# Lightning-AI/lit-llama

Hardware: NVIDIA H100
Metric: LLaMA-7B gptq.int4 decode tokens/sec (higher is better)
Workload: dtype bf16

## Files before the change

### lit-llama_b200/csrc/api.cu

```cuda
#include <algorithm>
#include <cstdlib>
#include <mutex>
#include <utility>
#include <vector>

#include "b2l_common.cuh"

namespace b2l {

extern void* g_attn_timeline;
int decode_step_persistent(const b2l_decode_args* d, b2l_stream_t stream);
int check_adapter_prefix(const b2l_adapter_prefix* pre, const char* who);
int check_lora(const b2l_lora* lo, int N, int K, const char* who);

static thread_local char g_err[512] = "";

void set_error(const char* fmt, ...) {
  va_list ap;
  va_start(ap, fmt);
  vsnprintf(g_err, sizeof(g_err), fmt, ap);
  va_end(ap);
}

int cuda_fail(cudaError_t e, const char* what) {
// ... 34 lines not shown
  if (cc_minor) *cc_minor = c;
  return 0;
}

struct PfWindow { const void* ptr[B2L_PF_SEGMENTS]; unsigned long long bytes[B2L_PF_SEGMENTS]; };

static size_t prefetch_distance() {
  static const long mb = [] { const char* e = getenv("B2L_PF_MB"); return e ? atol(e) : 0L; }();
  return mb > 0 ? (size_t)mb << 20 : 0;
}

static std::vector<PfWindow> prefetch_windows(const b2l_decode_args* d) {
  std::vector<std::pair<const uint8_t*, size_t>> ops;
  const bool w8 = (d->flags & B2L_F_W8) != 0;
  auto add = [&](const b2l_q4_weight& w) {
    ops.push_back({(const uint8_t*)w.qw_mma, w8 ? b2l_w8_tiled_i8_bytes(w.N, w.K) : b2l_q4_tiled_i8_bytes(w.N, w.K)});
  };
  for (int l = 0; l < d->n_layer; ++l) {
    add(d->layers[l].c_attn); add(d->layers[l].c_proj); add(d->layers[l].c_fc12); add(d->layers[l].mlp_proj);
  }
  add(d->lm_head);
  const size_t n = ops.size(), D = prefetch_distance();
  std::vector<PfWindow> out(n, PfWindow{});
  if (D == 0) return out;
  std::vector<size_t> start(n + 1, 0);
  for (size_t j = 0; j < n; ++j) start[j + 1] = start[j] + ops[j].second;
  for (size_t j = 0; j < n; ++j) {
    size_t lo = std::max(start[j] + D, start[j + 1]), hi = start[j + 1] + D;
    int sg = 0;
    size_t k = j + 1;
    size_t base = start[j + 1];
    while (lo < hi && sg < B2L_PF_SEGMENTS && k < j + 1 + n) {
      const auto& op = ops[k % n];
      const size_t op_lo = base, op_hi = base + op.second;
      if (lo < op_hi) {
        const size_t a = (lo - op_lo) & ~(size_t)127, b = std::min(hi, op_hi) - op_lo;
        if (b > a && op.first != nullptr) {
          out[j].ptr[sg] = op.first + a;
          out[j].bytes[sg] = (b - a + 15) & ~(size_t)15;
          ++sg;
        }
        lo = std::min(hi, op_hi);
      }
      base = op_hi;
      ++k;
    }
  }
  return out;
}

static int q4_call(const b2l_q4_weight& w, const void* x, int ldx, void* y, int ldy, int M, int sz_dtype, int prologue,
                   const void* norm_scale, float eps, int epilogue, const void* res, int ldres, int flags,
                   b2l_stream_t stream, void* trace = nullptr, void* batch_work = nullptr, const PfWindow* pf = nullptr,
                   const b2l_decode_args* kv_of = nullptr, int kv_layer = 0, const b2l_out_affine* aff = nullptr) {
  b2l_q4_linear_args a{};
  if (aff != nullptr) a.out_affine = *aff;
  if (kv_of != nullptr) {
    const int hs = kv_of->n_embd / kv_of->n_head;
    a.pf_kv[0] = kv_of->layers[kv_layer].k_cache; a.pf_kv[1] = kv_of->layers[kv_layer].v_cache;
    a.pf_rows = (const long long*)kv_of->input_pos;
    a.pf_rows_max = kv_of->S; a.pf_nseg = kv_of->B * kv_of->n_head; a.pf_row_bytes = hs * 2;
    a.pf_seg_stride = (unsigned long long)kv_of->S * hs * 2;
  }
  if (pf != nullptr)
    for (int i = 0; i < B2L_PF_SEGMENTS; ++i) { a.pf_ptr[i] = pf->ptr[i]; a.pf_bytes[i] = pf->bytes[i]; }
  a.x = x; a.ldx = ldx;
  const bool gemv = (M == 1 && w.qw_mma != nullptr);
  const bool batch = (!gemv && M <= 8 && w.qw_mma != nullptr && batch_work != nullptr);
  a.qw_tiled = (gemv || batch) ? w.qw_mma : w.qw_tiled; a.scales = w.scales; a.zeros = w.zeros; a.sz_dtype = sz_dtype;
  a.y = y; a.ldy = ldy;
  a.M = M; a.N = w.N; a.K = w.K;
  a.prologue = prologue; a.norm_scale = norm_scale; a.eps = eps;
  a.epilogue = epilogue; a.res = res; a.ldres = ldres;
  a.split_k = 0;
  a.flags = flags;
  a.trace = gemv ? trace : nullptr;
  if ((flags & B2L_F_Q4_BATCH_I8) && M > 1) {
    a.qw_tiled = w.qw_mma; a.trace = nullptr; a.workspace = batch_work;
    a.flags = flags & B2L_F_PDL;
    return b2l_q4_gemv_batch_i8(&a, stream);
  }
  if (flags & B2L_F_W8) {
    if (M > 1) {
      a.qw_tiled = w.qw_mma; a.trace = nullptr; a.workspace = batch_work;
      a.flags = flags & B2L_F_PDL;
      return b2l_w8_gemv_batch(&a, stream);
    }
    a.flags = flags & (B2L_F_PDL | B2L_F_DEBUG_NOCOMPUTE);
    return b2l_w8_gemv(&a, stream);
  }
  if (gemv) return b2l_q4_gemv(&a, stream);
  if (batch) {
    a.workspace = batch_work;
    return b2l_q4_gemv_batch(&a, stream);
  }
  if (a.qw_tiled == nullptr) {
    set_error("b2l_decode_step: weight has no tiling for batch %d", M);
    return B2L_E_STATE;
  }
  return b2l_q4_linear_tc(&a, stream);
}

static int q8_call(const b2l_decode_args* d, const b2l_q8_weight& w, const b2l_q8_weight* w2, const void* x, void* y,
                   const void* norm_scale, int epilogue, const void* res, const b2l_out_affine* aff, b2l_stream_t stream) {
  b2l_q8_linear_args a{};
  a.x = x; a.cb = w.cb; a.scb = w.scb;
  if (w2 != nullptr) { a.cb2 = w2->cb; a.scb2 = w2->scb; }
  a.y = y; a.N = w.N; a.K = w.K; a.threshold = d->q8_threshold;
  a.prologue = norm_scale != nullptr ? B2L_PRO_RMSNORM : B2L_PRO_NONE; a.norm_scale = norm_scale; a.eps = d->eps;
  a.epilogue = epilogue; a.res = res;
  if (aff != nullptr) a.out_affine = *aff;
  a.flags = d->flags & B2L_F_PDL;
  if (d->flags & B2L_F_Q8_BATCH)
    return b2l_q8_linear_batch(&a, d->B, d->batch_work, b2l_q8_linear_batch_workspace_bytes(w.K, d->B), stream);
  return b2l_q8_linear(&a, stream);
}
// ... 77 lines not shown
  if (d->flags & B2L_F_W8_BATCH) {
    B2L_CHECK_SUPPORTED(d->flags & B2L_F_W8, "b2l_decode_step: B2L_F_W8_BATCH needs B2L_F_W8 (gptq.int8)");
    B2L_CHECK_SUPPORTED(d->B >= 2 && d->B <= 16, "b2l_decode_step: B2L_F_W8_BATCH runs batches of 2..16, got B=%d", d->B);
    B2L_CHECK_SUPPORTED(d->plan == nullptr, "b2l_decode_step: B2L_F_W8_BATCH does not run in the persistent kernel (plan must be NULL)");
    B2L_CHECK_SUPPORTED(d->affines == nullptr && d->lm_head_affine.scale == nullptr && d->lm_head_affine.bias == nullptr,
                        "b2l_decode_step: B2L_F_W8_BATCH does not apply LLaMA-Adapter v2 affines (batch 1 only)");
    B2L_CHECK_ARG(d->batch_work != nullptr, "b2l_decode_step: B2L_F_W8_BATCH needs batch_work (b2l_w8_gemv_batch_workspace_bytes(max K, B) bytes)");
  } else if (d->flags & B2L_F_W8) {
    B2L_CHECK_SUPPORTED(d->B == 1, "b2l_decode_step: B2L_F_W8 (gptq.int8) runs batch 1 only, got B=%d", d->B);
    B2L_CHECK_SUPPORTED(d->plan == nullptr, "b2l_decode_step: B2L_F_W8 (gptq.int8) does not run in the persistent kernel (plan must be NULL)");
  }
  if (d->adapters != nullptr) {
    for (int l = 0; l < d->n_layer; ++l) {
      if (d->adapters[l].len == 0) continue;
      B2L_CHECK_SUPPORTED(d->plan == nullptr, "b2l_decode_step: adapters do not run in the persistent kernel (plan must be NULL)");
      if (int rc = check_adapter_prefix(&d->adapters[l], "b2l_decode_step")) return rc;
    }
  }
  if (d->loras != nullptr) {
    for (int l = 0; l < d->n_layer; ++l) {
      if (d->loras[l].r == 0) continue;
      B2L_CHECK_SUPPORTED(d->plan == nullptr, "b2l_decode_step: LoRA layers do not run in the persistent kernel (plan must be NULL)");
      if (int rc = check_lora(&d->loras[l], 3 * d->n_embd, d->n_embd, "b2l_decode_step")) return rc;
    }
  }
  const bool any_affine = d->affines != nullptr || d->lm_head_affine.scale != nullptr || d->lm_head_affine.bias != nullptr;
  if (any_affine) {
    B2L_CHECK_SUPPORTED(d->B == 1 || (d->flags & B2L_F_Q8_BATCH),
                        "b2l_decode_step: LLaMA-Adapter v2 affines run at batch 1 only, got B=%d", d->B);
    B2L_CHECK_SUPPORTED(d->plan == nullptr, "b2l_decode_step: LLaMA-Adapter v2 affines do not run in the persistent kernel (plan must be NULL)");
    B2L_CHECK_SUPPORTED(d->loras == nullptr, "b2l_decode_step: LLaMA-Adapter v2 affines and LoRA do not combine");
    auto ok = [](const b2l_out_affine& f) { return (f.scale == nullptr) == (f.bias == nullptr); };
    B2L_CHECK_ARG(ok(d->lm_head_affine), "b2l_decode_step: lm_head_affine needs both scale and bias (or neither)");
    B2L_CHECK_SUPPORTED(q8 || d->lm_head.qw_mma != nullptr, "b2l_decode_step: affines need the batch-1 tiling (qw_mma) of every weight");
    for (int l = 0; d->affines != nullptr && l < d->n_layer; ++l) {
      const b2l_layer_affine& f = d->affines[l];
      B2L_CHECK_ARG(ok(f.c_attn) && ok(f.c_proj) && ok(f.c_fc12) && ok(f.mlp_proj),
                    "b2l_decode_step: affines[%d] needs both scale and bias (or neither) per linear", l);
      const b2l_layer& L = d->layers[l];
      B2L_CHECK_SUPPORTED(q8 || (L.c_attn.qw_mma && L.c_proj.qw_mma && L.c_fc12.qw_mma && L.mlp_proj.qw_mma),
                          "b2l_decode_step: affines need the batch-1 tiling (qw_mma) of every weight");
    }
  }
  if (d->plan != nullptr) return decode_step_persistent(d, stream);
  const int C = d->n_embd, hs = C / d->n_head, B = d->B;
  const int fl = d->flags & ~B2L_F_ROW_POS;
  const int afl = d->flags & ~(B2L_F_W8 | B2L_F_Q8 | B2L_F_W8_BATCH | B2L_F_Q4_BATCH_I8 | B2L_F_Q8_BATCH);
  int rc;
  char* tlb = (char*)d->timeline;
  int li = 0;
  auto tl = [&]() -> void* { void* r = tlb ? (void*)(tlb + 512 * li) : nullptr; ++li; return r; };
  std::vector<PfWindow> pfw;
  if (B == 1 && d->lm_head.qw_mma != nullptr) pfw = prefetch_windows(d);
  static const int kv_prefetch = [] { const char* e = getenv("B2L_KV_PREFETCH"); return e ? atoi(e) : 0; }();
  const bool kv_ok = B == 1 && hs == 128 && d->lm_head.qw_mma != nullptr;
  int oi = 0;
  auto pf = [&]() -> const PfWindow* { const PfWindow* r = pfw.empty() ? nullptr : &pfw[oi]; ++oi; return r; };
  if ((rc = row_pos ? b2l_ring_advance_rows(d->input_pos, B, d->ring_start, d->S, stream)
                    : b2l_ring_advance(d->input_pos, 1, d->ring_start, d->S, stream)))
    return rc;
  if ((rc = b2l_embedding(d->idx, d->idx_is_i64, d->wte, d->x, B, C, d->vocab, stream))) return rc;
  for (int l = 0; l < d->n_layer; ++l) {
    const b2l_layer& L = d->layers[l];
    const b2l_layer_affine* af = d->affines != nullptr ? &d->affines[l] : nullptr;
    const b2l_q8_layer* Q = q8 ? &d->q8_layers[l] : nullptr;
    void* t = tl();
    if ((rc = Q ? q8_call(d, Q->c_attn, nullptr, d->x, d->qkv, L.rms_1, B2L_EPI_STORE, nullptr, af ? &af->c_attn : nullptr, stream)
                : q4_call(L.c_attn, d->x, C, d->qkv, 3 * C, B, d->sz_dtype, B2L_PRO_RMSNORM, L.rms_1, d->eps, B2L_EPI_STORE,
                          nullptr, 0, fl, stream, t, d->batch_work, pf(), (kv_ok && kv_prefetch == 2) ? d : nullptr, l,
                          af ? &af->c_attn : nullptr)))
      return rc;
    if (d->loras != nullptr && d->loras[l].r != 0 &&
        (rc = b2l_lora_apply(&d->loras[l], d->x, C, L.rms_1, d->eps, d->qkv, 3 * C, B, 3 * C, C, fl & B2L_F_PDL, stream)))
      return rc;
    g_attn_timeline = tl();
    const b2l_adapter_prefix* pre = (d->adapters != nullptr && d->adapters[l].len != 0) ? &d->adapters[l] : nullptr;
    if ((rc = pre != nullptr
                  ? b2l_attention_adapter(d->qkv, L.k_cache, L.v_cache, d->rope, d->input_pos, d->ring_start, d->att,
                                          d->attn_work, B, 1, d->n_head, hs, d->S, d->block_size, afl, pre, stream)
                  : b2l_attention(d->qkv, L.k_cache, L.v_cache, d->rope, d->input_pos, d->ring_start, d->att,
                                  d->attn_work, B, 1, d->n_head, hs, d->S, d->block_size, afl, stream))) {
      g_attn_timeline = nullptr;
      return rc;
    }
    g_attn_timeline = nullptr;
    t = tl();
    if ((rc = Q ? q8_call(d, Q->c_proj, nullptr, d->att, d->x, nullptr, B2L_EPI_RESIDUAL, d->x, af ? &af->c_proj : nullptr, stream)
                : q4_call(L.c_proj, d->att, C, d->x, C, B, d->sz_dtype, B2L_PRO_NONE, nullptr, 0.f, B2L_EPI_RESIDUAL, d->x, C,
                          fl, stream, t, d->batch_work, pf(), nullptr, 0, af ? &af->c_proj : nullptr)))
      return rc;
    t = tl();
    if ((rc = Q ? q8_call(d, Q->c_fc1, &Q->c_fc2, d->x, d->hid, L.rms_2, B2L_EPI_SWIGLU, nullptr, af ? &af->c_fc12 : nullptr, stream)
                : q4_call(L.c_fc12, d->x, C, d->hid, d->n_hidden, B, d->sz_dtype, B2L_PRO_RMSNORM, L.rms_2, d->eps,
                          B2L_EPI_SWIGLU, nullptr, 0, fl, stream, t, d->batch_work, pf(), nullptr, 0, af ? &af->c_fc12 : nullptr)))
      return rc;
    const bool kvpf = kv_prefetch == 1 && kv_ok && l + 1 < d->n_layer;
    t = tl();
    if ((rc = Q ? q8_call(d, Q->mlp_proj, nullptr, d->hid, d->x, nullptr, B2L_EPI_RESIDUAL, d->x, af ? &af->mlp_proj : nullptr, stream)
                : q4_call(L.mlp_proj, d->hid, d->n_hidden, d->x, C, B, d->sz_dtype, B2L_PRO_NONE, nullptr, 0.f,
                          B2L_EPI_RESIDUAL, d->x, C, fl, stream, t, d->batch_work, pf(), kvpf ? d : nullptr, l + 1,
                          af ? &af->mlp_proj : nullptr)))
      return rc;
  }
  if (q8) return q8_call(d, d->q8_lm_head, nullptr, d->x, d->logits, d->ln_f, B2L_EPI_STORE, nullptr, &d->lm_head_affine, stream);
  return q4_call(d->lm_head, d->x, C, d->logits, d->vocab, B, d->sz_dtype, B2L_PRO_RMSNORM, d->ln_f, d->eps,
                 B2L_EPI_STORE, nullptr, 0, fl, stream, tl(), d->batch_work, pf(), nullptr, 0, &d->lm_head_affine);
}
```

### lit-llama_b200/csrc/attention.cu

```cuda
#include <cstdlib>

#include "b2l_common.cuh"

namespace b2l {

__global__ void ring_advance_kernel(const int64_t* __restrict__ input_pos, int T, int32_t* ring_start, int S) {
  if (threadIdx.x == 0 && blockIdx.x == 0) {
    if (input_pos[T - 1] >= (int64_t)S) *ring_start = (*ring_start + 1) % S;
  }
}

__global__ void ring_advance_rows_kernel(const int64_t* __restrict__ input_pos, int B, int32_t* ring_start, int S) {
  for (int b = threadIdx.x; b < B; b += blockDim.x) {
    if (input_pos[b] >= (int64_t)S) ring_start[b] = (ring_start[b] + 1) % S;
  }
}

__global__ void rope_append_kernel(__nv_bfloat16* __restrict__ qkv, __nv_bfloat16* __restrict__ k_cache,
                                   __nv_bfloat16* __restrict__ v_cache, const float* __restrict__ rope,
                                   const int64_t* __restrict__ input_pos, const int32_t* __restrict__ ring_start,
                                   int T, int n_head, int hs, int S, int block_size, int rope_rows, int pos_stride) {
  const int bt = blockIdx.x, h = blockIdx.y, b = bt / T, t = bt % T;
  const int C = n_head * hs;
  long long p = input_pos ? input_pos[b * pos_stride + t] : (long long)t;
// ... 110 lines not shown
  __syncthreads();
  float M = -INFINITY;
#pragma unroll
  for (int w = 0; w < ATT_WARPS; ++w) M = fmaxf(M, sm_m[w]);
  float Ls = 0.f;
  float wgt[ATT_WARPS];
#pragma unroll
  for (int w = 0; w < ATT_WARPS; ++w) {
    wgt[w] = (sm_m[w] == -INFINITY) ? 0.f : __expf(sm_m[w] - M);
    Ls += sm_l[w] * wgt[w];
  }
  if (threadIdx.x == 0) { out[0] = M; out[1] = Ls; }
  for (int d = threadIdx.x; d < hs; d += blockDim.x) {
    float a = 0.f;
#pragma unroll
    for (int w = 0; w < ATT_WARPS; ++w) a += sm_acc[w][d] * wgt[w];
    out[2 + d] = a;
  }
}

__global__ void attn_combine_kernel(const float* __restrict__ work, __nv_bfloat16* __restrict__ y, int T,
                                    int n_head, int hs, int n_split) {
  pdl_launch_dependents();
  const int bh = blockIdx.x, b = bh / n_head, h = bh % n_head, t = blockIdx.y;
  const float* base = work + ((size_t)bh * T + t) * n_split * (hs + 2);
  float M = -INFINITY;
  for (int s = 0; s < n_split; ++s) M = fmaxf(M, base[(size_t)s * (hs + 2)]);
  float Ls = 0.f;
  for (int s = 0; s < n_split; ++s) {
    float ms = base[(size_t)s * (hs + 2)];
    if (ms != -INFINITY) Ls += base[(size_t)s * (hs + 2) + 1] * __expf(ms - M);
  }
  const float inv = 1.0f / Ls;
  __nv_bfloat16* yr = y + ((size_t)b * T + t) * (n_head * hs) + h * hs;
  for (int d = threadIdx.x; d < hs; d += blockDim.x) {
    float a = 0.f;
    for (int s = 0; s < n_split; ++s) {
      float ms = base[(size_t)s * (hs + 2)];
      if (ms != -INFINITY) a += base[(size_t)s * (hs + 2) + 2 + d] * __expf(ms - M);
    }
    yr[d] = f2bf(a * inv);
  }
}

__global__ void kv_unroll_kernel(const __nv_bfloat16* __restrict__ cache, const int32_t* __restrict__ ring_start,
                                 __nv_bfloat16* __restrict__ out, int S, int hs, int n_head, int ring_stride) {
  const int ring = ring_start[(blockIdx.x / n_head) * ring_stride];
  const int phys = (blockIdx.y + ring) % S;
  const __nv_bfloat16* src = cache + ((size_t)blockIdx.x * S + phys) * hs;
  __nv_bfloat16* dst = out + ((size_t)blockIdx.x * S + blockIdx.y) * hs;
  for (int d = threadIdx.x; d < hs; d += blockDim.x) dst[d] = src[d];
}

constexpr int FD_CHUNK = 256;
constexpr int FD_SUB = 64;
constexpr int FD_WARPS = 8;
constexpr int FD_CTAS_PER_SM = 3;
constexpr int WS_CHUNK = FD_SUB;

__device__ __forceinline__ void bf16x8_to_f32(const uint4& u, float* f) {
  const uint32_t w[4] = {u.x, u.y, u.z, u.w};
#pragma unroll
  for (int i = 0; i < 4; ++i) {
    f[2 * i] = __uint_as_float(w[i] << 16);
    f[2 * i + 1] = __uint_as_float(w[i] & 0xffff0000u);
  }
}

__device__ __forceinline__ uint32_t fd_smem_u32(const void* p) { return (uint32_t)__cvta_generic_to_shared(p); }
__device__ __forceinline__ void fd_bulk(uint32_t dst, const void* src, uint32_t bytes, uint32_t bar) {
  asm volatile("cp.async.bulk.shared::cluster.global.mbarrier::complete_tx::bytes [%0], [%1], %2, [%3];" ::"r"(dst), "l"(src), "r"(bytes), "r"(bar) : "memory");
}

constexpr int FD_SUB_BYTES = FD_SUB * 128 * 2;
constexpr int FD_SMEM_BYTES = 4 * FD_SUB_BYTES + FD_WARPS * 128 * 4 + 2 * FD_WARPS * 4 + 16;

__device__ __forceinline__ float fd_adapter_prefix(const float* sq, float* ssc, const __nv_bfloat16* __restrict__ ak,
                                                   const __nv_bfloat16* __restrict__ av, int alen, int warp, int lane,
                                                   int d, bool writer) {
  constexpr int HS = 128;
  const float4 qv = reinterpret_cast<const float4*>(sq)[lane];
#pragma unroll 2
  for (int j = warp; j < alen; j += FD_WARPS) {
    const uint2 ku = __ldg(reinterpret_cast<const uint2*>(ak + (size_t)j * HS) + lane);
    float s = qv.x * __uint_as_float(ku.x << 16);
    s = fmaf(qv.y, __uint_as_float(ku.x & 0xffff0000u), s);
    s = fmaf(qv.z, __uint_as_float(ku.y << 16), s);
    s = fmaf(qv.w, __uint_as_float(ku.y & 0xffff0000u), s);
    s = warp_sum(s);
    if (lane == 0) ssc[j] = s;
  }
  __syncthreads();
  float ay = 0.f;
  if (writer) {
    float mx = -INFINITY;
    for (int j = 0; j < alen; ++j) mx = fmaxf(mx, ssc[j]);
    float l = 0.f;
#pragma unroll 8
    for (int j = 0; j < alen; ++j) {
      const float p = __expf(ssc[j] - mx);
      l += p;
      ay = fmaf(p, bf2f(av[(size_t)j * HS + d]), ay);
    }
    ay /= l;
  }
  return ay;
}

__device__ __forceinline__ __nv_bfloat16 adapter_combine(float y, float ay, float gate) {
  return f2bf(rbf(y) + rbf(gate * rbf(ay)));
}

template <bool ADAPTER, bool ROWS>
__global__ void __launch_bounds__(FD_WARPS * 32, ADAPTER ? FD_CTAS_PER_SM : 0)
    attn_decode_fused_kernel(const __nv_bfloat16* qkv, __nv_bfloat16* __restrict__ k_cache,
                             __nv_bfloat16* __restrict__ v_cache, const float* __restrict__ rope,
                             const int64_t* __restrict__ input_pos, const int32_t* __restrict__ ring_start,
                             __nv_bfloat16* __restrict__ y, float* __restrict__ work, int* __restrict__ tickets,
                             int n_head, int S, int block_size, int n_split, unsigned long long* tl, int pre_tiles,
                             int smem_merge, int target_ctas, const __nv_bfloat16* __restrict__ pre_k,
                             const __nv_bfloat16* __restrict__ pre_v, const __nv_bfloat16* __restrict__ pre_gate,
                             int pre_len) {
  constexpr int HS = 128;
  extern __shared__ __align__(128) uint8_t fsm[];
  float* sm_acc = reinterpret_cast<float*>(fsm + 4 * FD_SUB_BYTES);
  float* sm_m = sm_acc + FD_WARPS * HS;
  float* sm_l = sm_m + FD_WARPS;
  unsigned long long* bars = reinterpret_cast<unsigned long long*>(sm_l + FD_WARPS);
  __shared__ int sm_last;

  if (threadIdx.x == 0) tl_min(tl, 0);
  const int bh = blockIdx.x, b = bh / n_head, h = bh % n_head, sp = blockIdx.y;
  unsigned long long* tl0 = (tl != nullptr && blockIdx.x == 0 && blockIdx.y == 0 && threadIdx.x == 0) ? tl + 8 : nullptr;
  int tli = 0;
  auto stamp = [&]() { if (tl0 != nullptr && tli < 24) tl0[tli++] = globaltimer_ns(); };
  stamp();
  const int lane = threadIdx.x & 31, warp = threadIdx.x >> 5;
  const int C = n_head * HS;
  const size_t head_base = ((size_t)b * n_head + h) * S * HS;

  const long long p = input_pos[ROWS ? b : 0];
  const int w_slot = (int)(p < S ? p : (long long)S - 1);
  const int L = w_slot + 1;
  const int want_splits = max(1, target_ctas / n_head);
  const int chunk = L <= FD_CHUNK ? FD_CHUNK
                                  : min(FD_CHUNK, max(FD_SUB, FD_SUB * ((L + FD_SUB * want_splits - 1) / (FD_SUB * want_splits))));
  const int n_active = (L + chunk - 1) / chunk;
  if (sp >= n_active) return;
  const int ring = ring_start[ROWS ? b : 0];
  const int j0 = sp * chunk, j1 = min(L, j0 + chunk);
  const int n_old = min(j1, L - 1) - j0;
  const int n_sub = (n_old + FD_SUB - 1) / FD_SUB;
  const bool has_new = (w_slot >= j0 && w_slot < j1);

  const uint32_t bar0 = fd_smem_u32(bars);
  auto request = [&](int i) {
    const int buf = i & 1;
    const int cnt = min(FD_SUB, n_old - i * FD_SUB);
    int phys0 = j0 + i * FD_SUB + ring; if (phys0 >= S) phys0 -= S;
    const int first = min(cnt, S - phys0);
    const uint32_t bar = bar0 + buf * 8;
    const uint32_t kd = fd_smem_u32(fsm) + buf * 2 * FD_SUB_BYTES, vd = kd + FD_SUB_BYTES;
    asm volatile("mbarrier.arrive.expect_tx.shared::cta.b64 _, [%0], %1;" ::"r"(bar), "r"((uint32_t)cnt * HS * 2 * 2) : "memory");
    fd_bulk(kd, k_cache + head_base + (size_t)phys0 * HS, (uint32_t)first * HS * 2, bar);
    fd_bulk(vd, v_cache + head_base + (size_t)phys0 * HS, (uint32_t)first * HS * 2, bar);
    if (first < cnt) {
      fd_bulk(kd + first * HS * 2, k_cache + head_base, (uint32_t)(cnt - first) * HS * 2, bar);
      fd_bulk(vd + first * HS * 2, v_cache + head_base, (uint32_t)(cnt - first) * HS * 2, bar);
    }
  };
  const int pre = (n_active == 1) ? 2 : pre_tiles;
  if (threadIdx.x == 0) {
    asm volatile("mbarrier.init.shared::cta.b64 [%0], 1;" ::"r"(bar0) : "memory");
    asm volatile("mbarrier.init.shared::cta.b64 [%0], 1;" ::"r"(bar0 + 8) : "memory");
    asm volatile("fence.mbarrier_init.release.cluster;" ::: "memory");
    if (n_sub > 0) request(0);
    if (pre > 1 && n_sub > 1) request(1);
  }
  if constexpr (ADAPTER) {
    if (threadIdx.x == 0) {
      const size_t off = (size_t)h * pre_len * HS;
      const uint32_t bytes = (uint32_t)pre_len * HS * 2;
      asm volatile("cp.async.bulk.prefetch.L2.global [%0], %1;" ::"l"(pre_k + off), "r"(bytes) : "memory");
      asm volatile("cp.async.bulk.prefetch.L2.global [%0], %1;" ::"l"(pre_v + off), "r"(bytes) : "memory");
    }
  }
  const long long prow = p < block_size ? p : (long long)block_size - 1;
  const int grp = lane >> 3, sub = lane & 7, d0 = sub * 16;
  float cs[16];
  {
    const float4* rp = reinterpret_cast<const float4*>(rope + ((size_t)prow * (HS / 2) + d0 / 2) * 2);
#pragma unroll
    for (int i = 0; i < 4; ++i) {
      float4 t = rp[i];
      cs[4 * i] = t.x; cs[4 * i + 1] = t.y; cs[4 * i + 2] = t.z; cs[4 * i + 3] = t.w;
    }
  }
  __syncthreads();
  pdl_wait();
  if (threadIdx.x == 0) tl_max(tl, 1);
  stamp();
  pdl_launch_dependents();

  const __nv_bfloat16* qrow = qkv + (size_t)b * 3 * C + h * HS + d0;
  float q[16];
  {
    float raw[16];
    const uint4 qa = ld_coherent_u4(qrow), qb = ld_coherent_u4(qrow + 8);
    if (threadIdx.x == 0 && pre <= 1 && n_sub > 1) request(1);
    bf16x8_to_f32(qa, raw);
    bf16x8_to_f32(qb, raw + 8);
    const float scale = rsqrtf((float)HS);
#pragma unroll
    for (int i = 0; i < 8; ++i) {
      const float c = cs[2 * i], s_ = cs[2 * i + 1];
      const float e = rbf(__fsub_rn(__fmul_rn(raw[2 * i], c), __fmul_rn(raw[2 * i + 1], s_)));
      const float o = rbf(__fadd_rn(__fmul_rn(raw[2 * i + 1], c), __fmul_rn(raw[2 * i], s_)));
      q[2 * i] = e * scale;
      q[2 * i + 1] = o * scale;
    }
  }
  float ay = 0.f;
  if constexpr (ADAPTER) {
    if (warp == 0 && grp == 0) {
      float4* dq = reinterpret_cast<float4*>(sm_acc + d0);
#pragma unroll
      for (int i = 0; i < 4; ++i) dq[i] = make_float4(q[4 * i], q[4 * i + 1], q[4 * i + 2], q[4 * i + 3]);
    }
    __syncthreads();
    ay = fd_adapter_prefix(sm_acc, sm_acc + HS, pre_k + (size_t)h * pre_len * HS, pre_v + (size_t)h * pre_len * HS,
                           pre_len, warp, lane, threadIdx.x & (HS - 1), threadIdx.x < HS);
  }

  float m = -INFINITY, l = 0.f, acc[16];
#pragma unroll
  for (int i = 0; i < 16; ++i) acc[i] = 0.f;
  if (tl0 != nullptr && q[0] != 12345.678f) stamp();
  if (has_new && warp == 0 && grp == 0) {
    int phys = w_slot + ring; if (phys >= S) phys -= S;
    float raw[16], kf[16], vf[16];
    bf16x8_to_f32(ld_coherent_u4(qrow + C), raw);
    bf16x8_to_f32(ld_coherent_u4(qrow + C + 8), raw + 8);
    uint32_t out[8];
#pragma unroll
    for (int i = 0; i < 8; ++i) {
      const float c = cs[2 * i], s_ = cs[2 * i + 1];
      kf[2 * i] = rbf(__fsub_rn(__fmul_rn(raw[2 * i], c), __fmul_rn(raw[2 * i + 1], s_)));
      kf[2 * i + 1] = rbf(__fadd_rn(__fmul_rn(raw[2 * i + 1], c), __fmul_rn(raw[2 * i], s_)));
      out[i] = (__float_as_uint(kf[2 * i]) >> 16) | (__float_as_uint(kf[2 * i + 1]) & 0xffff0000u);
    }
    const uint4 va = ld_coherent_u4(qrow + 2 * C), vb = ld_coherent_u4(qrow + 2 * C + 8);
    uint4* kd = reinterpret_cast<uint4*>(k_cache + head_base + (size_t)phys * HS + d0);
    uint4* vd = reinterpret_cast<uint4*>(v_cache + head_base + (size_t)phys * HS + d0);
    kd[0] = make_uint4(out[0], out[1], out[2], out[3]); kd[1] = make_uint4(out[4], out[5], out[6], out[7]);
    vd[0] = va; vd[1] = vb;
    bf16x8_to_f32(va, vf); bf16x8_to_f32(vb, vf + 8);
    float sc = 0.f;
#pragma unroll
    for (int e = 0; e < 16; ++e) sc = fmaf(q[e], kf[e], sc);
    sc += __shfl_xor_sync(0x000000ffu, sc, 1);
    sc += __shfl_xor_sync(0x000000ffu, sc, 2);
    sc += __shfl_xor_sync(0x000000ffu, sc, 4);
    const float mn = fmaxf(m, sc);
    const float corr = __expf(m - mn), pj = __expf(sc - mn);
    l = l * corr + pj;
#pragma unroll
    for (int e = 0; e < 16; ++e) acc[e] = fmaf(pj, vf[e], acc[e] * corr);
    m = mn;
  }
  for (int i = 0; i < n_sub; ++i) {
    const int buf = i & 1;
    const int cnt = min(FD_SUB, n_old - i * FD_SUB);
    {
      uint32_t ok;
      const uint32_t par = (uint32_t)(i >> 1) & 1u;
      do {
        asm volatile("{\n\t.reg .pred p;\n\tmbarrier.try_wait.parity.shared::cta.b64 p, [%1], %2;\n\tselp.u32 %0, 1, 0, p;\n\t}" : "=r"(ok) : "r"(bar0 + buf * 8), "r"(par) : "memory");
      } while (!ok);
    }
    const __nv_bfloat16* kt = reinterpret_cast<const __nv_bfloat16*>(fsm + buf * 2 * FD_SUB_BYTES);
    const __nv_bfloat16* vt = kt + FD_SUB * HS;
    stamp();
    float sc[2];
    bool valid[2];
    const uint4* vr[2];
#pragma unroll
    for (int it = 0; it < 2; ++it) {
      const int r = warp * 8 + it * 4 + grp;
      valid[it] = r < cnt;
      const int rc = valid[it] ? r : 0;
      const uint4* kr = reinterpret_cast<const uint4*>(kt + (size_t)rc * HS + d0);
      vr[it] = reinterpret_cast<const uint4*>(vt + (size_t)rc * HS + d0);
      float kf[16];
      bf16x8_to_f32(kr[0], kf); bf16x8_to_f32(kr[1], kf + 8);
      float a0 = 0.f, a1 = 0.f;
#pragma unroll
      for (int e = 0; e < 8; ++e) { a0 = fmaf(q[e], kf[e], a0); a1 = fmaf(q[8 + e], kf[8 + e], a1); }
      sc[it] = a0 + a1;
    }
#pragma unroll
    for (int o = 1; o <= 4; o <<= 1) {
      sc[0] += __shfl_xor_sync(0xffffffffu, sc[0], o);
      sc[1] += __shfl_xor_sync(0xffffffffu, sc[1], o);
    }
    {
      const float s0 = valid[0] ? sc[0] : -INFINITY, s1 = valid[1] ? sc[1] : -INFINITY;
      const float mn = fmaxf(m, fmaxf(s0, s1));
      if (mn != -INFINITY) {
        const float corr = __expf(m - mn), p0 = __expf(s0 - mn), p1 = __expf(s1 - mn);
        float v0[16], v1[16];
        bf16x8_to_f32(vr[0][0], v0); bf16x8_to_f32(vr[0][1], v0 + 8);
        bf16x8_to_f32(vr[1][0], v1); bf16x8_to_f32(vr[1][1], v1 + 8);
        l = l * corr + p0 + p1;
#pragma unroll
        for (int e = 0; e < 16; ++e) acc[e] = fmaf(p1, v1[e], fmaf(p0, v0[e], acc[e] * corr));
        m = mn;
      }
    }
    __syncthreads();
    stamp();
    if (threadIdx.x == 0 && i + 2 < n_sub) request(i + 2);
  }
  if (threadIdx.x == 0) tl_max(tl, 2);
  __syncwarp();
  if (threadIdx.x == 0) tl_max(tl, 3);
  float* part = reinterpret_cast<float*>(fsm);
  float* pm = part + 32 * HS;
  float* pl = pm + 32, *pw = pl + 32;
  const int n_part = smem_merge ? 32 : FD_WARPS;
  if (smem_merge) {
    const int g = warp * 4 + grp;
    float4* dst = reinterpret_cast<float4*>(part + g * HS + d0);
#pragma unroll
    for (int i = 0; i < 4; ++i) dst[i] = make_float4(acc[4 * i], acc[4 * i + 1], acc[4 * i + 2], acc[4 * i + 3]);
    if (sub == 0) { pm[g] = m; pl[g] = l; }
  } else {
#pragma unroll
    for (int off = 8; off <= 16; off <<= 1) {
      const float mo = __shfl_xor_sync(0xffffffffu, m, off);
      const float lo = __shfl_xor_sync(0xffffffffu, l, off);
      const float mn = fmaxf(m, mo);
      const float ca = (m == -INFINITY) ? 0.f : __expf(m - mn);
      const float cb = (mo == -INFINITY) ? 0.f : __expf(mo - mn);
      l = l * ca + lo * cb;
#pragma unroll
      for (int i = 0; i < 16; ++i) {
        const float ao = __shfl_xor_sync(0xffffffffu, acc[i], off);
        acc[i] = acc[i] * ca + ao * cb;
      }
      m = mn;
    }
    if (lane == 0) { pm[warp] = m; pl[warp] = l; }
    if (grp == 0) {
      float4* dst = reinterpret_cast<float4*>(part + warp * HS + d0);
#pragma unroll
      for (int i = 0; i < 4; ++i) dst[i] = make_float4(acc[4 * i], acc[4 * i + 1], acc[4 * i + 2], acc[4 * i + 3]);
    }
  }
  __syncthreads();
  if (warp == 0) {
    const float mi = lane < n_part ? pm[lane] : -INFINITY;
    const float Mx = warp_max(mi);
    const float wi = (mi == -INFINITY) ? 0.f : __expf(mi - Mx);
    const float Lx = warp_sum(lane < n_part ? pl[lane] * wi : 0.f);
    pw[lane] = wi;
    if (lane == 0) { pw[32] = Mx; pw[33] = Lx; }
  }
  __syncthreads();
  const float M = pw[32], Ls = pw[33];
  const int d = threadIdx.x & (HS - 1);
  const bool writer = threadIdx.x < HS;
  float a = 0.f;
  if (writer) {
#pragma unroll 8
    for (int g = 0; g < n_part; ++g) a = fmaf(part[g * HS + d], pw[g], a);
  }
  stamp();
  if (n_active == 1) {
    if constexpr (ADAPTER) {
      if (writer) y[(size_t)b * C + h * HS + d] = adapter_combine(a / Ls, ay, bf2f(pre_gate[h]));
    } else {
      if (writer) y[(size_t)b * C + h * HS + d] = f2bf(a / Ls);
    }
    if (threadIdx.x == 0) tl_max(tl, 4);
    stamp();
    return;
  }
  float* out = work + ((size_t)bh * n_split + sp) * (HS + 2);
  if (threadIdx.x == 0) { out[0] = M; out[1] = Ls; }
  if (writer) out[2 + d] = a;
  __syncthreads();
  if (threadIdx.x == 0) {
    int t;
    asm volatile("atom.add.acq_rel.gpu.global.s32 %0, [%1], 1;" : "=r"(t) : "l"(tickets + bh) : "memory");
    sm_last = (t == n_active - 1);
    if (sm_last) tickets[bh] = 0;
  }
  __syncthreads();
  stamp();
  if (!sm_last) return;
  const float* base = work + (size_t)bh * n_split * (HS + 2);
  float MM = -INFINITY, LL = 0.f, aa = 0.f;
  for (int s0 = 0; s0 < n_active; s0 += 8) {
    float ms[8], ls[8], as[8];
#pragma unroll
    for (int i = 0; i < 8; ++i) {
      const int s2 = s0 + i;
      const bool ok = s2 < n_active;
      const float* bp = base + (size_t)(ok ? s2 : s0) * (HS + 2);
      ms[i] = ok ? __ldcg(bp) : -INFINITY;
// ... 287 lines not shown

using namespace b2l;

static inline size_t ws_partials_bytes(int B, int n_head, int head_size, int T, int S) {
  int n_split, chunk;
  split_plan(T, S, &n_split, &chunk);
  size_t a = (size_t)B * n_head * T * n_split * (head_size + 2) * sizeof(float);
  size_t f = (size_t)B * n_head * ((S + WS_CHUNK - 1) / WS_CHUNK) * (head_size + 2) * sizeof(float);
  return ((a > f ? a : f) + 15) & ~(size_t)15;
}

extern "C" size_t b2l_attn_workspace_bytes(int B, int n_head, int head_size, int T, int S) {
  return ws_partials_bytes(B, n_head, head_size, T, S) + (size_t)B * n_head * sizeof(int);
}

extern "C" int b2l_ring_advance(const int64_t* input_pos, int T, int32_t* ring_start, int S, b2l_stream_t stream) {
  B2L_CHECK_ARG(input_pos && ring_start && T > 0 && S > 0, "b2l_ring_advance: bad argument");
  ring_advance_kernel<<<1, 32, 0, (cudaStream_t)stream>>>(input_pos, T, ring_start, S);
  B2L_LAUNCH_CHECK("ring_advance_kernel");
  return 0;
}

extern "C" int b2l_ring_advance_rows(const int64_t* input_pos, int B, int32_t* ring_start, int S, b2l_stream_t stream) {
  B2L_CHECK_ARG(input_pos && ring_start, "b2l_ring_advance_rows: null pointer");
  B2L_CHECK_ARG(B > 0 && S > 0, "b2l_ring_advance_rows: bad shape (B=%d, S=%d)", B, S);
  ring_advance_rows_kernel<<<1, 32, 0, (cudaStream_t)stream>>>(input_pos, B, ring_start, S);
  B2L_LAUNCH_CHECK("ring_advance_rows_kernel");
  return 0;
}

static int launch_adapter_prefix(const void* qkv, const b2l_adapter_prefix* pre, void* y, int B, int T, int n_head,
                                 int head_size, cudaStream_t st) {
  attn_adapter_prefix_kernel<<<dim3(B * T, n_head), ATT_WARPS * 32, 0, st>>>(
      (const __nv_bfloat16*)qkv, (const __nv_bfloat16*)pre->k, (const __nv_bfloat16*)pre->v,
      (const __nv_bfloat16*)pre->gate, (__nv_bfloat16*)y, n_head, head_size, pre->len);
  B2L_LAUNCH_CHECK("attn_adapter_prefix_kernel");
  return 0;
}

static int check_row_pos(int flags, int T, const char* who) {
  if (!(flags & B2L_F_ROW_POS)) return 0;
  B2L_CHECK_SUPPORTED(T == 1, "%s: B2L_F_ROW_POS runs one token per row (T == 1), got T=%d", who, T);
  B2L_CHECK_SUPPORTED(!(flags & B2L_F_ROPE_ROWS), "%s: B2L_F_ROW_POS does not combine with B2L_F_ROPE_ROWS", who);
  return 0;
}

static int attention_impl(void* qkv, void* k_cache, void* v_cache, const void* rope, const int64_t* input_pos,
                          const int32_t* ring_start, void* y, void* work, int B, int T, int n_head, int head_size,
                          int S, int block_size, int flags, const b2l_adapter_prefix* pre, cudaStream_t st) {
  const int pos_stride = (flags & B2L_F_ROW_POS) ? 1 : 0;
  if (T == 1 && head_size == 128 && !(flags & B2L_F_ROPE_ROWS) && !(flags & B2L_F_ATTN_UNFUSED)) {
    const int n_split = (S + FD_SUB - 1) / FD_SUB;
    int* tickets = reinterpret_cast<int*>(reinterpret_cast<char*>(work) + ws_partials_bytes(B, n_head, head_size, T, S));
    static const int env_pre = [] { const char* e = getenv("B2L_ATTN_PRE"); return e ? atoi(e) : 1; }();
    static const int env_smem_merge = [] { const char* e = getenv("B2L_ATTN_SMEM_MERGE"); return e ? atoi(e) : 0; }();
    LaunchCfg lc(dim3(B * n_head, n_split), dim3(FD_WARPS * 32), FD_SMEM_BYTES, st, (flags & B2L_F_PDL) != 0);
    static DynSmemCache smem_cache[2][2];
    auto launch = [&](auto kernel, const b2l_adapter_prefix* pf) -> int {
      if (int rc = ensure_dyn_smem(kernel, FD_SMEM_BYTES, smem_cache[pf != nullptr][pos_stride])) return rc;
      B2L_CUDA(cudaLaunchKernelEx(&lc.cfg, kernel, (const __nv_bfloat16*)qkv, (__nv_bfloat16*)k_cache,
                                  (__nv_bfloat16*)v_cache, (const float*)rope, input_pos, ring_start, (__nv_bfloat16*)y,
                                  (float*)work, tickets, n_head, S, block_size, n_split, (unsigned long long*)g_attn_timeline, env_pre, env_smem_merge,
                                  FD_CTAS_PER_SM * sm_count(), (const __nv_bfloat16*)(pf ? pf->k : nullptr),
                                  (const __nv_bfloat16*)(pf ? pf->v : nullptr), (const __nv_bfloat16*)(pf ? pf->gate : nullptr),
                                  pf ? pf->len : 0));
      return 0;
    };
    if (pre == nullptr)
      return pos_stride ? launch(attn_decode_fused_kernel<false, true>, nullptr) : launch(attn_decode_fused_kernel<false, false>, nullptr);
    return pos_stride ? launch(attn_decode_fused_kernel<true, true>, pre) : launch(attn_decode_fused_kernel<true, false>, pre);
  }
  int rt = head_size / 2 < 32 ? 32 : head_size / 2;
  rope_append_kernel<<<dim3(B * T, n_head), rt, 0, st>>>((__nv_bfloat16*)qkv, (__nv_bfloat16*)k_cache,
                                                        (__nv_bfloat16*)v_cache, (const float*)rope, input_pos,
                                                        ring_start, T, n_head, head_size, S, block_size, (flags & B2L_F_ROPE_ROWS) ? 1 : 0,
                                                        pos_stride);
  B2L_LAUNCH_CHECK("rope_append_kernel");
  KvView kv{(const __nv_bfloat16*)k_cache, (const __nv_bfloat16*)v_cache, (size_t)n_head * S * head_size,
            (size_t)S * head_size, (size_t)head_size, S};
  if (int rc = launch_attn((const __nv_bfloat16*)qkv, kv, input_pos, ring_start, (float*)work, (__nv_bfloat16*)y, B, T,
                           n_head, head_size, S, pos_stride, st))
    return rc;
  return pre == nullptr ? 0 : launch_adapter_prefix(qkv, pre, y, B, T, n_head, head_size, st);
}

extern "C" int b2l_attention(void* qkv, void* k_cache, void* v_cache, const void* rope, const int64_t* input_pos,
                             const int32_t* ring_start, void* y, void* work, int B, int T, int n_head,
                             int head_size, int S, int block_size, int flags, b2l_stream_t stream) {
  B2L_CHECK_ARG(qkv && k_cache && v_cache && rope && input_pos && ring_start && y && work,
                "b2l_attention: null pointer");
  B2L_CHECK_ARG(B > 0 && T > 0 && n_head > 0 && S > 0 && T <= S && block_size > 0, "b2l_attention: bad shape");
  B2L_CHECK_SUPPORTED(head_size % 2 == 0 && head_size >= 2 && head_size <= 32 * ATT_MAX_EPL,
                      "b2l_attention: head_size %d unsupported (even, <= %d)", head_size, 32 * ATT_MAX_EPL);
  if (int rc = check_row_pos(flags, T, "b2l_attention")) return rc;
  return attention_impl(qkv, k_cache, v_cache, rope, input_pos, ring_start, y, work, B, T, n_head, head_size, S,
                        block_size, flags, nullptr, (cudaStream_t)stream);
}

extern "C" int b2l_attention_adapter(void* qkv, void* k_cache, void* v_cache, const void* rope,
                                     const int64_t* input_pos, const int32_t* ring_start, void* y, void* work, int B,
                                     int T, int n_head, int head_size, int S, int block_size, int flags,
                                     const b2l_adapter_prefix* prefix, b2l_stream_t stream) {
  B2L_CHECK_ARG(qkv && k_cache && v_cache && rope && input_pos && ring_start && y && work,
                "b2l_attention_adapter: null pointer");
  B2L_CHECK_ARG(B > 0 && T > 0 && n_head > 0 && S > 0 && T <= S && block_size > 0, "b2l_attention_adapter: bad shape");
  B2L_CHECK_SUPPORTED(head_size % 2 == 0 && head_size >= 2 && head_size <= 32 * ATT_MAX_EPL,
                      "b2l_attention_adapter: head_size %d unsupported (even, <= %d)", head_size, 32 * ATT_MAX_EPL);
  if (int rc = check_row_pos(flags, T, "b2l_attention_adapter")) return rc;
  if (int rc = check_adapter_prefix(prefix, "b2l_attention_adapter")) return rc;
  return attention_impl(qkv, k_cache, v_cache, rope, input_pos, ring_start, y, work, B, T, n_head, head_size, S,
                        block_size, flags, prefix, (cudaStream_t)stream);
}

static int attention_nocache_impl(void* qkv, const void* rope, void* y, void* work, int B, int T, int n_head,
                                  int head_size, int block_size, cudaStream_t st) {
// ... 52 lines not shown
```

Before: 587.6.

## Deepen attention decode K/V ring to three stages and drop env-driven variants

The fused decode attention kernel now uses a three-slot K/V bulk-copy ring with mbarrier parity tracking instead of double buffering. It prefetches two tiles up front and skips the per-tile __syncthreads when no further refill is needed. Per-CTA chunk size is no longer capped at 256 rows, and the target is two CTAs per SM instead of three. The larger shared memory footprint trades occupancy for deeper copy pipelining. The unused KV-prefetch and smem-merge environment options are removed, which is mainly cleanup.

```diff
diff --git a/lit-llama_b200/csrc/api.cu b/lit-llama_b200/csrc/api.cu
--- a/lit-llama_b200/csrc/api.cu
+++ b/lit-llama_b200/csrc/api.cu
@@ -110,16 +110,9 @@
 static int q4_call(const b2l_q4_weight& w, const void* x, int ldx, void* y, int ldy, int M, int sz_dtype, int prologue,
                    const void* norm_scale, float eps, int epilogue, const void* res, int ldres, int flags,
                    b2l_stream_t stream, void* trace = nullptr, void* batch_work = nullptr, const PfWindow* pf = nullptr,
-                   const b2l_decode_args* kv_of = nullptr, int kv_layer = 0, const b2l_out_affine* aff = nullptr) {
+                   const b2l_out_affine* aff = nullptr) {
   b2l_q4_linear_args a{};
   if (aff != nullptr) a.out_affine = *aff;
-  if (kv_of != nullptr) {
-    const int hs = kv_of->n_embd / kv_of->n_head;
-    a.pf_kv[0] = kv_of->layers[kv_layer].k_cache; a.pf_kv[1] = kv_of->layers[kv_layer].v_cache;
-    a.pf_rows = (const long long*)kv_of->input_pos;
-    a.pf_rows_max = kv_of->S; a.pf_nseg = kv_of->B * kv_of->n_head; a.pf_row_bytes = hs * 2;
-    a.pf_seg_stride = (unsigned long long)kv_of->S * hs * 2;
-  }
   if (pf != nullptr)
     for (int i = 0; i < B2L_PF_SEGMENTS; ++i) { a.pf_ptr[i] = pf->ptr[i]; a.pf_bytes[i] = pf->bytes[i]; }
   a.x = x; a.ldx = ldx;
@@ -303,8 +296,6 @@
   auto tl = [&]() -> void* { void* r = tlb ? (void*)(tlb + 512 * li) : nullptr; ++li; return r; };
   std::vector<PfWindow> pfw;
   if (B == 1 && d->lm_head.qw_mma != nullptr) pfw = prefetch_windows(d);
-  static const int kv_prefetch = [] { const char* e = getenv("B2L_KV_PREFETCH"); return e ? atoi(e) : 0; }();
-  const bool kv_ok = B == 1 && hs == 128 && d->lm_head.qw_mma != nullptr;
   int oi = 0;
   auto pf = [&]() -> const PfWindow* { const PfWindow* r = pfw.empty() ? nullptr : &pfw[oi]; ++oi; return r; };
   if ((rc = row_pos ? b2l_ring_advance_rows(d->input_pos, B, d->ring_start, d->S, stream)
@@ -318,7 +309,7 @@
     void* t = tl();
     if ((rc = Q ? q8_call(d, Q->c_attn, nullptr, d->x, d->qkv, L.rms_1, B2L_EPI_STORE, nullptr, af ? &af->c_attn : nullptr, stream)
                 : q4_call(L.c_attn, d->x, C, d->qkv, 3 * C, B, d->sz_dtype, B2L_PRO_RMSNORM, L.rms_1, d->eps, B2L_EPI_STORE,
-                          nullptr, 0, fl, stream, t, d->batch_work, pf(), (kv_ok && kv_prefetch == 2) ? d : nullptr, l,
+                          nullptr, 0, fl, stream, t, d->batch_work, pf(),
                           af ? &af->c_attn : nullptr)))
       return rc;
     if (d->loras != nullptr && d->loras[l].r != 0 &&
@@ -338,22 +329,21 @@
     t = tl();
     if ((rc = Q ? q8_call(d, Q->c_proj, nullptr, d->att, d->x, nullptr, B2L_EPI_RESIDUAL, d->x, af ? &af->c_proj : nullptr, stream)
                 : q4_call(L.c_proj, d->att, C, d->x, C, B, d->sz_dtype, B2L_PRO_NONE, nullptr, 0.f, B2L_EPI_RESIDUAL, d->x, C,
-                          fl, stream, t, d->batch_work, pf(), nullptr, 0, af ? &af->c_proj : nullptr)))
+                          fl, stream, t, d->batch_work, pf(), af ? &af->c_proj : nullptr)))
       return rc;
     t = tl();
     if ((rc = Q ? q8_call(d, Q->c_fc1, &Q->c_fc2, d->x, d->hid, L.rms_2, B2L_EPI_SWIGLU, nullptr, af ? &af->c_fc12 : nullptr, stream)
                 : q4_call(L.c_fc12, d->x, C, d->hid, d->n_hidden, B, d->sz_dtype, B2L_PRO_RMSNORM, L.rms_2, d->eps,
-                          B2L_EPI_SWIGLU, nullptr, 0, fl, stream, t, d->batch_work, pf(), nullptr, 0, af ? &af->c_fc12 : nullptr)))
-      return rc;
-    const bool kvpf = kv_prefetch == 1 && kv_ok && l + 1 < d->n_layer;
+                          B2L_EPI_SWIGLU, nullptr, 0, fl, stream, t, d->batch_work, pf(), af ? &af->c_fc12 : nullptr)))
+      return rc;
     t = tl();
     if ((rc = Q ? q8_call(d, Q->mlp_proj, nullptr, d->hid, d->x, nullptr, B2L_EPI_RESIDUAL, d->x, af ? &af->mlp_proj : nullptr, stream)
                 : q4_call(L.mlp_proj, d->hid, d->n_hidden, d->x, C, B, d->sz_dtype, B2L_PRO_NONE, nullptr, 0.f,
-                          B2L_EPI_RESIDUAL, d->x, C, fl, stream, t, d->batch_work, pf(), kvpf ? d : nullptr, l + 1,
+                          B2L_EPI_RESIDUAL, d->x, C, fl, stream, t, d->batch_work, pf(),
                           af ? &af->mlp_proj : nullptr)))
       return rc;
   }
   if (q8) return q8_call(d, d->q8_lm_head, nullptr, d->x, d->logits, d->ln_f, B2L_EPI_STORE, nullptr, &d->lm_head_affine, stream);
   return q4_call(d->lm_head, d->x, C, d->logits, d->vocab, B, d->sz_dtype, B2L_PRO_RMSNORM, d->ln_f, d->eps,
-                 B2L_EPI_STORE, nullptr, 0, fl, stream, tl(), d->batch_work, pf(), nullptr, 0, &d->lm_head_affine);
-}
+                 B2L_EPI_STORE, nullptr, 0, fl, stream, tl(), d->batch_work, pf(), &d->lm_head_affine);
+}
diff --git a/lit-llama_b200/csrc/attention.cu b/lit-llama_b200/csrc/attention.cu
--- a/lit-llama_b200/csrc/attention.cu
+++ b/lit-llama_b200/csrc/attention.cu
@@ -186,10 +186,12 @@
   for (int d = threadIdx.x; d < hs; d += blockDim.x) dst[d] = src[d];
 }
 
-constexpr int FD_CHUNK = 256;
+constexpr int FD_ONE_CTA = 256;
 constexpr int FD_SUB = 64;
+constexpr int FD_RING = 3;
+constexpr int FD_PRE = 2;
 constexpr int FD_WARPS = 8;
-constexpr int FD_CTAS_PER_SM = 3;
+constexpr int FD_CTAS_PER_SM = 2;
 constexpr int WS_CHUNK = FD_SUB;
 
 __device__ __forceinline__ void bf16x8_to_f32(const uint4& u, float* f) {
@@ -207,7 +209,8 @@
 }
 
 constexpr int FD_SUB_BYTES = FD_SUB * 128 * 2;
-constexpr int FD_SMEM_BYTES = 4 * FD_SUB_BYTES + FD_WARPS * 128 * 4 + 2 * FD_WARPS * 4 + 16;
+constexpr int FD_SMEM_BYTES = FD_RING * 2 * FD_SUB_BYTES + FD_WARPS * 128 * 4 + 2 * FD_WARPS * 4 + 8 * FD_RING;
+static_assert(32 * 128 * 4 + 35 * 4 <= FD_RING * 2 * FD_SUB_BYTES, "the CTA merge reuses the idle K / V ring");
 
 __device__ __forceinline__ float fd_adapter_prefix(const float* sq, float* ssc, const __nv_bfloat16* __restrict__ ak,
                                                    const __nv_bfloat16* __restrict__ av, int alen, int warp, int lane,
@@ -251,13 +254,13 @@
                              __nv_bfloat16* __restrict__ v_cache, const float* __restrict__ rope,
                              const int64_t* __restrict__ input_pos, const int32_t* __restrict__ ring_start,
                              __nv_bfloat16* __restrict__ y, float* __restrict__ work, int* __restrict__ tickets,
-                             int n_head, int S, int block_size, int n_split, unsigned long long* tl, int pre_tiles,
-                             int smem_merge, int target_ctas, const __nv_bfloat16* __restrict__ pre_k,
+                             int n_head, int S, int block_size, int n_split, unsigned long long* tl,
+                             int target_ctas, const __nv_bfloat16* __restrict__ pre_k,
                              const __nv_bfloat16* __restrict__ pre_v, const __nv_bfloat16* __restrict__ pre_gate,
                              int pre_len) {
   constexpr int HS = 128;
   extern __shared__ __align__(128) uint8_t fsm[];
-  float* sm_acc = reinterpret_cast<float*>(fsm + 4 * FD_SUB_BYTES);
+  float* sm_acc = reinterpret_cast<float*>(fsm + FD_RING * 2 * FD_SUB_BYTES);
   float* sm_m = sm_acc + FD_WARPS * HS;
   float* sm_l = sm_m + FD_WARPS;
   unsigned long long* bars = reinterpret_cast<unsigned long long*>(sm_l + FD_WARPS);
@@ -277,8 +280,7 @@
   const int w_slot = (int)(p < S ? p : (long long)S - 1);
   const int L = w_slot + 1;
   const int want_splits = max(1, target_ctas / n_head);
-  const int chunk = L <= FD_CHUNK ? FD_CHUNK
-                                  : min(FD_CHUNK, max(FD_SUB, FD_SUB * ((L + FD_SUB * want_splits - 1) / (FD_SUB * want_splits))));
+  const int chunk = L <= FD_ONE_CTA ? FD_ONE_CTA : FD_SUB * ((L + FD_SUB * want_splits - 1) / (FD_SUB * want_splits));
   const int n_active = (L + chunk - 1) / chunk;
   if (sp >= n_active) return;
   const int ring = ring_start[ROWS ? b : 0];
@@ -289,7 +291,7 @@
 
   const uint32_t bar0 = fd_smem_u32(bars);
   auto request = [&](int i) {
-    const int buf = i & 1;
+    const int buf = i % FD_RING;
     const int cnt = min(FD_SUB, n_old - i * FD_SUB);
     int phys0 = j0 + i * FD_SUB + ring; if (phys0 >= S) phys0 -= S;
     const int first = min(cnt, S - phys0);
@@ -303,13 +305,13 @@
       fd_bulk(vd + first * HS * 2, v_cache + head_base, (uint32_t)(cnt - first) * HS * 2, bar);
     }
   };
-  const int pre = (n_active == 1) ? 2 : pre_tiles;
+  const int n_ring = min(n_sub, FD_RING);
+  const int n_pre = n_active == 1 ? n_ring : min(n_sub, FD_PRE);
   if (threadIdx.x == 0) {
-    asm volatile("mbarrier.init.shared::cta.b64 [%0], 1;" ::"r"(bar0) : "memory");
-    asm volatile("mbarrier.init.shared::cta.b64 [%0], 1;" ::"r"(bar0 + 8) : "memory");
+#pragma unroll
+    for (int i = 0; i < FD_RING; ++i) asm volatile("mbarrier.init.shared::cta.b64 [%0], 1;" ::"r"(bar0 + 8 * i) : "memory");
     asm volatile("fence.mbarrier_init.release.cluster;" ::: "memory");
-    if (n_sub > 0) request(0);
-    if (pre > 1 && n_sub > 1) request(1);
+    for (int i = 0; i < n_pre; ++i) request(i);
   }
   if constexpr (ADAPTER) {
     if (threadIdx.x == 0) {
@@ -341,7 +343,8 @@
   {
     float raw[16];
     const uint4 qa = ld_coherent_u4(qrow), qb = ld_coherent_u4(qrow + 8);
-    if (threadIdx.x == 0 && pre <= 1 && n_sub > 1) request(1);
+    if (threadIdx.x == 0)
+      for (int i = n_pre; i < n_ring; ++i) request(i);
     bf16x8_to_f32(qa, raw);
     bf16x8_to_f32(qb, raw + 8);
     const float scale = rsqrtf((float)HS);
@@ -403,11 +406,11 @@
     m = mn;
   }
   for (int i = 0; i < n_sub; ++i) {
-    const int buf = i & 1;
+    const int buf = i % FD_RING;
     const int cnt = min(FD_SUB, n_old - i * FD_SUB);
     {
       uint32_t ok;
-      const uint32_t par = (uint32_t)(i >> 1) & 1u;
+      const uint32_t par = (uint32_t)(i / FD_RING) & 1u;
       do {
         asm volatile("{\n\t.reg .pred p;\n\tmbarrier.try_wait.parity.shared::cta.b64 p, [%1], %2;\n\tselp.u32 %0, 1, 0, p;\n\t}" : "=r"(ok) : "r"(bar0 + buf * 8), "r"(par) : "memory");
       } while (!ok);
@@ -451,45 +454,40 @@
         m = mn;
       }
     }
-    __syncthreads();
-    stamp();
-    if (threadIdx.x == 0 && i + 2 < n_sub) request(i + 2);
-  }
+    if (i + FD_RING < n_sub) {
+      __syncthreads();
+      stamp();
+      if (threadIdx.x == 0) request(i + FD_RING);
+    }
+  }
+  __syncthreads();
   if (threadIdx.x == 0) tl_max(tl, 2);
   __syncwarp();
   if (threadIdx.x == 0) tl_max(tl, 3);
   float* part = reinterpret_cast<float*>(fsm);
   float* pm = part + 32 * HS;
   float* pl = pm + 32, *pw = pl + 32;
-  const int n_part = smem_merge ? 32 : FD_WARPS;
-  if (smem_merge) {
-    const int g = warp * 4 + grp;
-    float4* dst = reinterpret_cast<float4*>(part + g * HS + d0);
+  const int n_part = FD_WARPS;
+#pragma unroll
+  for (int off = 8; off <= 16; off <<= 1) {
+    const float mo = __shfl_xor_sync(0xffffffffu, m, off);
+    const float lo = __shfl_xor_sync(0xffffffffu, l, off);
+    const float mn = fmaxf(m, mo);
+    const float ca = (m == -INFINITY) ? 0.f : __expf(m - mn);
+    const float cb = (mo == -INFINITY) ? 0.f : __expf(mo - mn);
+    l = l * ca + lo * cb;
+#pragma unroll
+    for (int i = 0; i < 16; ++i) {
+      const float ao = __shfl_xor_sync(0xffffffffu, acc[i], off);
+      acc[i] = acc[i] * ca + ao * cb;
+    }
+    m = mn;
+  }
+  if (lane == 0) { pm[warp] = m; pl[warp] = l; }
+  if (grp == 0) {
+    float4* dst = reinterpret_cast<float4*>(part + warp * HS + d0);
 #pragma unroll
     for (int i = 0; i < 4; ++i) dst[i] = make_float4(acc[4 * i], acc[4 * i + 1], acc[4 * i + 2], acc[4 * i + 3]);
-    if (sub == 0) { pm[g] = m; pl[g] = l; }
-  } else {
-#pragma unroll
-    for (int off = 8; off <= 16; off <<= 1) {
-      const float mo = __shfl_xor_sync(0xffffffffu, m, off);
-      const float lo = __shfl_xor_sync(0xffffffffu, l, off);
-      const float mn = fmaxf(m, mo);
-      const float ca = (m == -INFINITY) ? 0.f : __expf(m - mn);
-      const float cb = (mo == -INFINITY) ? 0.f : __expf(mo - mn);
-      l = l * ca + lo * cb;
-#pragma unroll
-      for (int i = 0; i < 16; ++i) {
-        const float ao = __shfl_xor_sync(0xffffffffu, acc[i], off);
-        acc[i] = acc[i] * ca + ao * cb;
-      }
-      m = mn;
-    }
-    if (lane == 0) { pm[warp] = m; pl[warp] = l; }
-    if (grp == 0) {
-      float4* dst = reinterpret_cast<float4*>(part + warp * HS + d0);
-#pragma unroll
-      for (int i = 0; i < 4; ++i) dst[i] = make_float4(acc[4 * i], acc[4 * i + 1], acc[4 * i + 2], acc[4 * i + 3]);
-    }
   }
   __syncthreads();
   if (warp == 0) {
@@ -883,15 +881,13 @@
   if (T == 1 && head_size == 128 && !(flags & B2L_F_ROPE_ROWS) && !(flags & B2L_F_ATTN_UNFUSED)) {
     const int n_split = (S + FD_SUB - 1) / FD_SUB;
     int* tickets = reinterpret_cast<int*>(reinterpret_cast<char*>(work) + ws_partials_bytes(B, n_head, head_size, T, S));
-    static const int env_pre = [] { const char* e = getenv("B2L_ATTN_PRE"); return e ? atoi(e) : 1; }();
-    static const int env_smem_merge = [] { const char* e = getenv("B2L_ATTN_SMEM_MERGE"); return e ? atoi(e) : 0; }();
     LaunchCfg lc(dim3(B * n_head, n_split), dim3(FD_WARPS * 32), FD_SMEM_BYTES, st, (flags & B2L_F_PDL) != 0);
     static DynSmemCache smem_cache[2][2];
     auto launch = [&](auto kernel, const b2l_adapter_prefix* pf) -> int {
       if (int rc = ensure_dyn_smem(kernel, FD_SMEM_BYTES, smem_cache[pf != nullptr][pos_stride])) return rc;
       B2L_CUDA(cudaLaunchKernelEx(&lc.cfg, kernel, (const __nv_bfloat16*)qkv, (__nv_bfloat16*)k_cache,
                                   (__nv_bfloat16*)v_cache, (const float*)rope, input_pos, ring_start, (__nv_bfloat16*)y,
-                                  (float*)work, tickets, n_head, S, block_size, n_split, (unsigned long long*)g_attn_timeline, env_pre, env_smem_merge,
+                                  (float*)work, tickets, n_head, S, block_size, n_split, (unsigned long long*)g_attn_timeline,
                                   FD_CTAS_PER_SM * sm_count(), (const __nv_bfloat16*)(pf ? pf->k : nullptr),
                                   (const __nv_bfloat16*)(pf ? pf->v : nullptr), (const __nv_bfloat16*)(pf ? pf->gate : nullptr),
                                   pf ? pf->len : 0));
```

Measured after the change: 594.3, median of 6. 1.1% higher.
